# filthyrake/vlog

Hardware: AMD Instinct MI355X
Metric: audio-sec transcribed per wall-sec (RTFx), large-v3, 1/2/4/8 MI355X; WER delta (higher is better)
Workload: dtype bf16; 1 GPU; config 4: large-v3 bf16 greedy, timestamps on, 150 x 30 s windows per GPU of the seeded speech-like corpus (uniform transcript lengths), window-sharded; model=large-v3, windows_per_gpu=150, decoder_steps=113, decode=all-rows batch, decoder_row_steps=16950, corpus=uniform, parallelism=window-shard x1

## Files before the change

### vlog_amd/csrc/attn_enc.hip

```cpp
#include "common.h"
#include <cstdlib>
#include <stdexcept>
#include <string>
#include <type_traits>

#define HD 64
#define KT 64
#define VT_LD 68

__device__ __forceinline__ int kswz(int row, int ch) { return row * HD + ((ch ^ ((row >> 1) & 7)) << 3); }

__global__ __launch_bounds__(256) void attn_enc_kernel(const bf16* __restrict__ qkv, bf16* __restrict__ out, int T,
                                                       int d, float scale_log2) {
  __shared__ __attribute__((aligned(16))) bf16 sK[KT * HD];
  __shared__ __attribute__((aligned(16))) bf16 sVt[HD * VT_LD];
  const int tid = threadIdx.x, lane = tid & 63, wv = tid >> 6;
  const int g = lane >> 4, ql = lane & 15;
  const int h = blockIdx.y, b = blockIdx.z;
  const long long ld = 3LL * d;
  const bf16* base = qkv + (long long)b * T * ld;
  const int q0 = blockIdx.x * 64 + wv * 16;

  bf16x8 qf[2];
  {
    const int q = q0 + ql;
#pragma unroll
    for (int kk = 0; kk < 2; ++kk) {
      if (q < T) qf[kk] = *(const bf16x8*)(base + (long long)q * ld + h * HD + kk * 32 + 8 * g);
      else qf[kk] = bf16x8{};
    }
  }

  f32x4 o[4];
#pragma unroll
  for (int i = 0; i < 4; ++i) o[i] = f32x4{0.f, 0.f, 0.f, 0.f};
  float m_run = -INFINITY, l_run = 0.f;

  i32x4 rk[2], rv[2];
  const int nt = (T + KT - 1) / KT;
#define LOAD_TILE(t_)                                                                       \
  {                                                                                         \
    _Pragma("unroll") for (int i = 0; i < 2; ++i) {                                         \
      const int c = tid + i * 256, key = (t_) * KT + (c >> 3), ch = c & 7;                  \
      if (key < T) {                                                                        \
        const bf16* p = base + (long long)key * ld + h * HD + ch * 8;                        \
        rk[i] = *(const i32x4*)(p + d);                                                     \
        rv[i] = *(const i32x4*)(p + 2 * d);                                                 \
      } else {                                                                              \
        rk[i] = i32x4{0, 0, 0, 0};                                                          \
        rv[i] = i32x4{0, 0, 0, 0};                                                          \
      }                                                                                     \
    }                                                                                       \
  }
  LOAD_TILE(0);
  for (int t = 0; t < nt; ++t) {
    __syncthreads();
#pragma unroll
    for (int i = 0; i < 2; ++i) {
      const int c = tid + i * 256, key = c >> 3, ch = c & 7;
      *(i32x4*)(&sK[kswz(key, ch)]) = rk[i];
      bf16x8 vv = __builtin_bit_cast(bf16x8, rv[i]);
#pragma unroll
      for (int e = 0; e < 8; ++e) sVt[(ch * 8 + e) * VT_LD + key] = vv[e];
    }
    __syncthreads();
    if (t + 1 < nt) LOAD_TILE(t + 1);

    f32x4 s[4];
#pragma unroll
    for (int mi = 0; mi < 4; ++mi) {
      s[mi] = f32x4{0.f, 0.f, 0.f, 0.f};
#pragma unroll
      for (int kk = 0; kk < 2; ++kk) {
        const bf16x8 ka = *(const bf16x8*)(&sK[kswz(mi * 16 + ql, kk * 4 + g)]);
        s[mi] = __builtin_amdgcn_mfma_f32_16x16x32_bf16(ka, qf[kk], s[mi], 0, 0, 0);
      }
    }
    float tmax = -INFINITY;
    const int kbase = t * KT;
#pragma unroll
    for (int mi = 0; mi < 4; ++mi)
#pragma unroll
      for (int e = 0; e < 4; ++e) {
        const int key = kbase + mi * 16 + 4 * g + e;
        float v = s[mi][e] * scale_log2;
        if (key >= T) v = -INFINITY;
        s[mi][e] = v;
        tmax = fmaxf(tmax, v);
      }
    tmax = fmaxf(tmax, __shfl_xor(tmax, 16, 64));
    tmax = fmaxf(tmax, __shfl_xor(tmax, 32, 64));
    const float m_new = fmaxf(m_run, tmax);
    const float alpha = exp2f(m_run - m_new);
    float psum = 0.f;
#pragma unroll
    for (int mi = 0; mi < 4; ++mi)
#pragma unroll
      for (int e = 0; e < 4; ++e) {
        const float p = exp2f(s[mi][e] - m_new);
        s[mi][e] = p;
        psum += p;
      }
    psum += __shfl_xor(psum, 16, 64);
    psum += __shfl_xor(psum, 32, 64);
    l_run = l_run * alpha + psum;
    m_run = m_new;
#pragma unroll
    for (int ni = 0; ni < 4; ++ni) o[ni] *= alpha;

#pragma unroll
    for (int ks = 0; ks < 2; ++ks) {
      bf16x8 pb;
#pragma unroll
      for (int e = 0; e < 4; ++e) {
        pb[e] = f2bf(s[2 * ks][e]);
        pb[4 + e] = f2bf(s[2 * ks + 1][e]);
      }
#pragma unroll
      for (int ni = 0; ni < 4; ++ni) {
        const bf16* vr = &sVt[(ni * 16 + ql) * VT_LD + ks * 32 + 4 * g];
        const bf16x4 lo = *(const bf16x4*)(vr);
        const bf16x4 hi = *(const bf16x4*)(vr + 16);
        bf16x8 va;
#pragma unroll
        for (int e = 0; e < 4; ++e) { va[e] = lo[e]; va[4 + e] = hi[e]; }
        o[ni] = __builtin_amdgcn_mfma_f32_16x16x32_bf16(va, pb, o[ni], 0, 0, 0);
      }
    }
  }
#undef LOAD_TILE

  const int q = q0 + ql;
  if (q < T) {
    const float inv = 1.0f / l_run;
    bf16* orow = out + ((long long)b * T + q) * d + h * HD;
#pragma unroll
    for (int ni = 0; ni < 4; ++ni) {
      bf16x4 w;
#pragma unroll
      for (int e = 0; e < 4; ++e) w[e] = f2bf(o[ni][e] * inv);
      *(bf16x4*)(orow + ni * 16 + 4 * g) = w;
    }
  }
}

#define A2_KT 64
#define A2_THR 8.0f
typedef __attribute__((ext_vector_type(4))) short i16x4;
typedef __attribute__((ext_vector_type(2))) int i32x2;

__device__ __forceinline__ int a2_kslot(int r, int c) { return r * 64 + ((c ^ ((r >> 1) & 7)) << 3); }
__device__ __forceinline__ int a2_vslot(int r, int c) { return r * 64 + ((c ^ (((r >> 1) & 1) << 2)) << 3); }

__global__ __launch_bounds__(256, 2) void attn_enc_v2_kernel(const bf16* __restrict__ qkv, bf16* __restrict__ out,
                                                             int T, int d, float scale_log2, int n_head) {
  __shared__ __attribute__((aligned(16))) bf16 smem[2 * 2 * A2_KT * HD];
  const int tid = threadIdx.x, lane = tid & 63, wv = tid >> 6;
  const int ql = lane & 31, hh = lane >> 5;
  const int nqt = (T + 127) / 128;
  int qt, h, b;
  {
    const int nwg = gridDim.x, bid = blockIdx.x, xcd = bid & 7, q8 = nwg >> 3, r8 = nwg & 7;
    const int wgid = (xcd < r8 ? xcd * (q8 + 1) : r8 * (q8 + 1) + (xcd - r8) * q8) + (bid >> 3);
    qt = wgid % nqt;
    const int rest = wgid / nqt;
    h = rest % n_head;
    b = rest / n_head;
  }
  const long long ld = 3LL * d;
  const bf16* base = qkv + (long long)b * T * ld + h * HD;
  const int q = qt * 128 + wv * 32 + ql;

  bf16x8 qf[4];
  {
    const int qc = min(q, T - 1);
#pragma unroll
    for (int s = 0; s < 4; ++s) {
      const bf16x8 v = *(const bf16x8*)(base + (long long)qc * ld + 16 * s + 8 * hh);
#pragma unroll
      for (int j = 0; j < 8; ++j) qf[s][j] = f2bf(bf2f(v[j]) * scale_log2);
    }
  }
  f32x16 o[2];
#pragma unroll
  for (int i = 0; i < 2; ++i)
#pragma unroll
    for (int r = 0; r < 16; ++r) o[i][r] = 0.f;
  float m_run = -INFINITY, l_run = 0.f;

  i32x4 rk[2], rv[2];
  const int nt = (T + A2_KT - 1) / A2_KT;
  auto load_tile = [&](int t) {
#pragma unroll
    for (int i = 0; i < 2; ++i) {
      const int c = tid + i * 256, key = min(t * A2_KT + (c >> 3), T - 1), ch = c & 7;
      const bf16* p = base + (long long)key * ld + ch * 8;
      rk[i] = *(const i32x4*)(p + d);
      rv[i] = *(const i32x4*)(p + 2 * d);
    }
  };
  auto store_tile = [&](int buf) {
    bf16* sK = smem + buf * (2 * A2_KT * HD);
    bf16* sV = sK + A2_KT * HD;
#pragma unroll
    for (int i = 0; i < 2; ++i) {
      const int c = tid + i * 256, r = c >> 3, ch = c & 7;
      *(i32x4*)(sK + a2_kslot(r, ch)) = rk[i];
      *(i32x4*)(sV + a2_vslot(r, ch)) = rv[i];
    }
  };
  load_tile(0);
  store_tile(0);
  __syncthreads();

  const int G = lane >> 4, gi = lane & 15, gq = gi >> 2, gp = gi & 3;
  for (int t = 0; t < nt; ++t) {
    const bf16* sK = smem + (t & 1) * (2 * A2_KT * HD);
    const bf16* sV = sK + A2_KT * HD;
    if (t + 1 < nt) load_tile(t + 1);

    f32x16 sc[2];
#pragma unroll
    for (int kb = 0; kb < 2; ++kb) {
#pragma unroll
      for (int r = 0; r < 16; ++r) sc[kb][r] = 0.f;
#pragma unroll
      for (int s = 0; s < 4; ++s) {
        const bf16x8 ka = *(const bf16x8*)(sK + a2_kslot(kb * 32 + ql, 2 * s + hh));
        sc[kb] = __builtin_amdgcn_mfma_f32_32x32x16_bf16(ka, qf[s], sc[kb], 0, 0, 0);
      }
    }
    if (t == nt - 1) {
#pragma unroll
      for (int kb = 0; kb < 2; ++kb)
#pragma unroll
        for (int r = 0; r < 16; ++r) {
          const int key = t * A2_KT + kb * 32 + 8 * (r >> 2) + 4 * hh + (r & 3);
          if (key >= T) sc[kb][r] = -INFINITY;
        }
    }
    float mx = sc[0][0];
#pragma unroll
    for (int kb = 0; kb < 2; ++kb)
#pragma unroll
      for (int r = 0; r < 16; ++r) mx = fmaxf(mx, sc[kb][r]);
    mx = fmaxf(mx, __shfl_xor(mx, 32, 64));
    if (__any(mx > m_run + A2_THR)) {
      const float mn = fmaxf(m_run, mx);
      const float alpha = __builtin_amdgcn_exp2f(m_run - mn);
      l_run *= alpha;
#pragma unroll
      for (int i = 0; i < 2; ++i)
#pragma unroll
        for (int r = 0; r < 16; ++r) o[i][r] *= alpha;
      m_run = mn;
    }
    bf16x8 pf[2][2];
#pragma unroll
    for (int kb = 0; kb < 2; ++kb)
#pragma unroll
      for (int r = 0; r < 16; ++r) {
        const float pv = __builtin_amdgcn_exp2f(sc[kb][r] - m_run);
        l_run += pv;
        pf[kb][r >> 3][r & 7] = f2bf(pv);
      }
#pragma unroll
    for (int kb = 0; kb < 2; ++kb)
#pragma unroll
      for (int s = 0; s < 2; ++s)
#pragma unroll
        for (int hb = 0; hb < 2; ++hb) {
          bf16x8 va;
#ifndef A2_SCALAR_V
          i32x2 vw[2];
#endif
#pragma unroll
          for (int jh = 0; jh < 2; ++jh) {
            const int row = kb * 32 + 16 * s + 8 * jh + 4 * (G >> 1) + gq;
            const int col = 32 * hb + 16 * (G & 1) + 4 * gp;
#ifdef A2_SCALAR_V
            const int rowb = row - gq, hdc = 32 * hb + 16 * (G & 1) + gi;
#pragma unroll
            for (int e = 0; e < 4; ++e) va[4 * jh + e] = sV[a2_vslot(rowb + e, hdc >> 3) + (hdc & 7)];
#else
            const bf16* ad = sV + a2_vslot(row, col >> 3) + (col & 7);
            vw[jh] = __builtin_bit_cast(i32x2, __builtin_amdgcn_ds_read_tr16_b64_v4i16(
                                                   (__attribute__((address_space(3))) i16x4*)(ad)));
#endif
          }
#ifndef A2_SCALAR_V
          va = __builtin_bit_cast(bf16x8, i32x4{vw[0][0], vw[0][1], vw[1][0], vw[1][1]});
#endif
          o[hb] = __builtin_amdgcn_mfma_f32_32x32x16_bf16(va, pf[kb][s], o[hb], 0, 0, 0);
        }
    if (t + 1 < nt) store_tile((t + 1) & 1);
    __syncthreads();
  }

  l_run += __shfl_xor(l_run, 32, 64);
  if (q < T) {
    const float inv = 1.0f / l_run;
    bf16* orow = out + ((long long)b * T + q) * d + h * HD;
#pragma unroll
    for (int hb = 0; hb < 2; ++hb)
#pragma unroll
      for (int g = 0; g < 4; ++g) {
        bf16x4 w;
#pragma unroll
        for (int e = 0; e < 4; ++e) w[e] = f2bf(o[hb][4 * g + e] * inv);
        *(bf16x4*)(orow + 32 * hb + 8 * g + 4 * hh) = w;
      }
  }
}

__device__ __forceinline__ void a3_scores(const bf16* sK, const bf16x8 (&qf)[4], int ql, int hh, f32x16 (&sc)[2]) {
#pragma unroll
  for (int kb = 0; kb < 2; ++kb)
#pragma unroll
    for (int r = 0; r < 16; ++r) sc[kb][r] = 0.f;
#pragma unroll
  for (int s = 0; s < 4; ++s)
#pragma unroll
    for (int kb = 0; kb < 2; ++kb) {
      const bf16x8 ka = *(const bf16x8*)(sK + a2_kslot(kb * 32 + ql, 2 * s + hh));
      sc[kb] = __builtin_amdgcn_mfma_f32_32x32x16_bf16(ka, qf[s], sc[kb], 0, 0, 0);
    }
}

__global__ __launch_bounds__(256, 2) void attn_enc_v3_kernel(const bf16* __restrict__ qkv, bf16* __restrict__ out,
                                                             int T, int d, float scale_log2, int n_head) {
  __shared__ __attribute__((aligned(16))) bf16 smem[3 * 2 * A2_KT * HD];
  const int tid = threadIdx.x, lane = tid & 63, wv = tid >> 6;
  const int ql = lane & 31, hh = lane >> 5;
  const int nqt = (T + 127) / 128;
  int qt, h, b;
  {
    const int nwg = gridDim.x, bid = blockIdx.x, xcd = bid & 7, q8 = nwg >> 3, r8 = nwg & 7;
    const int wgid = (xcd < r8 ? xcd * (q8 + 1) : r8 * (q8 + 1) + (xcd - r8) * q8) + (bid >> 3);
    qt = wgid % nqt;
    const int rest = wgid / nqt;
    h = rest % n_head;
    b = rest / n_head;
  }
  const long long ld = 3LL * d;
  const bf16* base = qkv + (long long)b * T * ld + h * HD;
  const int q = qt * 128 + wv * 32 + ql;

  bf16x8 qf[4];
  {
    const int qc = min(q, T - 1);
#pragma unroll
    for (int s = 0; s < 4; ++s) {
      const bf16x8 v = *(const bf16x8*)(base + (long long)qc * ld + 16 * s + 8 * hh);
#pragma unroll
      for (int j = 0; j < 8; ++j) qf[s][j] = f2bf(bf2f(v[j]) * scale_log2);
    }
  }
  f32x16 o[2];
#pragma unroll
  for (int i = 0; i < 2; ++i)
#pragma unroll
    for (int r = 0; r < 16; ++r) o[i][r] = 0.f;
  float m_run = -INFINITY, l_run = 0.f;

  i32x4 rk[2], rv[2];
  const int nt = (T + A2_KT - 1) / A2_KT;
  auto load_tile = [&](int t) {
#pragma unroll
    for (int i = 0; i < 2; ++i) {
      const int c = tid + i * 256, key = min(t * A2_KT + (c >> 3), T - 1), ch = c & 7;
      const bf16* p = base + (long long)key * ld + ch * 8;
      rk[i] = *(const i32x4*)(p + d);
      rv[i] = *(const i32x4*)(p + 2 * d);
    }
  };
  auto store_tile = [&](int slot) {
    bf16* sK = smem + slot * (2 * A2_KT * HD);
    bf16* sV = sK + A2_KT * HD;
#pragma unroll
    for (int i = 0; i < 2; ++i) {
      const int c = tid + i * 256, r = c >> 3, ch = c & 7;
      *(i32x4*)(sK + a2_kslot(r, ch)) = rk[i];
      *(i32x4*)(sV + a2_vslot(r, ch)) = rv[i];
    }
  };
  load_tile(0);
  store_tile(0);
  if (nt > 1) {
    load_tile(1);
    store_tile(1);
  }
  __syncthreads();

  const int G = lane >> 4, gi = lane & 15, gq = gi >> 2, gp = gi & 3;
  f32x16 sc[2];
  a3_scores(smem, qf, ql, hh, sc);

  auto tile = [&](int t, int slot, auto last_tag) {
    constexpr bool LAST = decltype(last_tag)::value;
    const bf16* sV = smem + slot * (2 * A2_KT * HD) + A2_KT * HD;
    f32x16 sn[2];
    if constexpr (!LAST) load_tile(t + 2);
    if constexpr (LAST) {
#pragma unroll
      for (int kb = 0; kb < 2; ++kb)
#pragma unroll
        for (int r = 0; r < 16; ++r) {
          const int key = t * A2_KT + kb * 32 + 8 * (r >> 2) + 4 * hh + (r & 3);
          if (key >= T) sc[kb][r] = -INFINITY;
        }
    }
    float mx = sc[0][0];
#pragma unroll
    for (int kb = 0; kb < 2; ++kb)
#pragma unroll
      for (int r = 0; r < 16; ++r) mx = fmaxf(mx, sc[kb][r]);
    mx = fmaxf(mx, __shfl_xor(mx, 32, 64));
    if (__any(mx > m_run + A2_THR)) {
      const float mn = fmaxf(m_run, mx);
      const float alpha = __builtin_amdgcn_exp2f(m_run - mn);
      l_run *= alpha;
#pragma unroll
      for (int i = 0; i < 2; ++i)
#pragma unroll
        for (int r = 0; r < 16; ++r) o[i][r] *= alpha;
      m_run = mn;
    }
    if constexpr (!LAST) a3_scores(smem + (slot == 2 ? 0 : slot + 1) * (2 * A2_KT * HD), qf, ql, hh, sn);
    bf16x8 pf[2][2];
#pragma unroll
    for (int kb = 0; kb < 2; ++kb)
#pragma unroll
      for (int r = 0; r < 16; ++r) {
        const float pv = __builtin_amdgcn_exp2f(sc[kb][r] - m_run);
        l_run += pv;
        pf[kb][r >> 3][r & 7] = f2bf(pv);
      }
#pragma unroll
    for (int kb = 0; kb < 2; ++kb)
#pragma unroll
      for (int s = 0; s < 2; ++s)
#pragma unroll
        for (int hb = 0; hb < 2; ++hb) {
          i32x2 vw[2];
#pragma unroll
          for (int jh = 0; jh < 2; ++jh) {
            const int row = kb * 32 + 16 * s + 8 * jh + 4 * (G >> 1) + gq;
            const int col = 32 * hb + 16 * (G & 1) + 4 * gp;
            const bf16* ad = sV + a2_vslot(row, col >> 3) + (col & 7);
            vw[jh] = __builtin_bit_cast(i32x2, __builtin_amdgcn_ds_read_tr16_b64_v4i16(
                                                   (__attribute__((address_space(3))) i16x4*)(ad)));
          }
          const bf16x8 va = __builtin_bit_cast(bf16x8, i32x4{vw[0][0], vw[0][1], vw[1][0], vw[1][1]});
          o[hb] = __builtin_amdgcn_mfma_f32_32x32x16_bf16(va, pf[kb][s], o[hb], 0, 0, 0);
        }
    if constexpr (!LAST) {
      store_tile(slot == 0 ? 2 : slot - 1);
      __syncthreads();
#pragma unroll
      for (int kb = 0; kb < 2; ++kb) sc[kb] = sn[kb];
    }
  };
  int slot = 0;
  for (int t = 0; t < nt - 1; ++t) {
    tile(t, slot, std::false_type{});
    slot = slot == 2 ? 0 : slot + 1;
  }
  tile(nt - 1, slot, std::true_type{});

  l_run += __shfl_xor(l_run, 32, 64);
  if (q < T) {
    const float inv = 1.0f / l_run;
    bf16* orow = out + ((long long)b * T + q) * d + h * HD;
#pragma unroll
    for (int hb = 0; hb < 2; ++hb)
#pragma unroll
      for (int g = 0; g < 4; ++g) {
        bf16x4 w;
#pragma unroll
        for (int e = 0; e < 4; ++e) w[e] = f2bf(o[hb][4 * g + e] * inv);
        *(bf16x4*)(orow + 32 * hb + 8 * g + 4 * hh) = w;
      }
  }
}

static int attn_enc_form() {
  static const int v = [] {
    const char* e1 = std::getenv("VLOG_AMD_ATTN_V1");
    if (e1 && e1[0] == '1') return 1;
    const char* e = std::getenv("VLOG_AMD_ATTN_V");
    const int f = e ? std::atoi(e) : 2;
    return (f >= 1 && f <= 3) ? f : 2;
  }();
  return v;
}

void launch_attn_enc(const bf16* qkv, bf16* out, int B, int T, int d, int n_head, hipStream_t st) {
  if (B <= 0) return;
  if (d != n_head * HD) throw std::runtime_error("attn_enc: head_dim must be 64");
  const float scale_log2 = 0.125f * 1.4426950408889634f;
  const int form = attn_enc_form();
  if (form == 1) {
    dim3 grid((T + 63) / 64, n_head, B);
    hipLaunchKernelGGL(attn_enc_kernel, grid, dim3(256), 0, st, qkv, out, T, d, scale_log2);
  } else {
    const long long nblk = (long long)((T + 127) / 128) * n_head * B;
    if (nblk > (1LL << 31) - 1) throw std::runtime_error("attn_enc: grid too large");
    if (form == 3)
      hipLaunchKernelGGL(attn_enc_v3_kernel, dim3((unsigned)nblk), dim3(256), 0, st, qkv, out, T, d, scale_log2, n_head);
    else
      hipLaunchKernelGGL(attn_enc_v2_kernel, dim3((unsigned)nblk), dim3(256), 0, st, qkv, out, T, d, scale_log2, n_head);
  }
  WM_LAUNCH_CHECK("attn_enc_kernel");
}
```

Before: 3888 audio_s/s.

## Add v4 encoder attention with buffer loads, double-buffering and tail skipping

Replaces the v1 and v3 encoder attention kernels with a new default v4 kernel. It loads K/V through buffer resource loads with scalar offsets, so clamping and bounds checks are done by the hardware. It uses a 2-slot LDS double buffer with compile-time buffer indices and drops v3's score prefetching. It also skips fully out-of-range waves and the unused half of the last key tile. Encoder time should drop through less address arithmetic and wasted tail work, but losing v3's score/PV overlap may reduce latency hiding.

```diff
diff --git a/vlog_amd/csrc/attn_enc.hip b/vlog_amd/csrc/attn_enc.hip
--- a/vlog_amd/csrc/attn_enc.hip
+++ b/vlog_amd/csrc/attn_enc.hip
@@ -5,144 +5,6 @@
 #include <type_traits>
 
 #define HD 64
-#define KT 64
-#define VT_LD 68
-
-__device__ __forceinline__ int kswz(int row, int ch) { return row * HD + ((ch ^ ((row >> 1) & 7)) << 3); }
-
-__global__ __launch_bounds__(256) void attn_enc_kernel(const bf16* __restrict__ qkv, bf16* __restrict__ out, int T,
-                                                       int d, float scale_log2) {
-  __shared__ __attribute__((aligned(16))) bf16 sK[KT * HD];
-  __shared__ __attribute__((aligned(16))) bf16 sVt[HD * VT_LD];
-  const int tid = threadIdx.x, lane = tid & 63, wv = tid >> 6;
-  const int g = lane >> 4, ql = lane & 15;
-  const int h = blockIdx.y, b = blockIdx.z;
-  const long long ld = 3LL * d;
-  const bf16* base = qkv + (long long)b * T * ld;
-  const int q0 = blockIdx.x * 64 + wv * 16;
-
-  bf16x8 qf[2];
-  {
-    const int q = q0 + ql;
-#pragma unroll
-    for (int kk = 0; kk < 2; ++kk) {
-      if (q < T) qf[kk] = *(const bf16x8*)(base + (long long)q * ld + h * HD + kk * 32 + 8 * g);
-      else qf[kk] = bf16x8{};
-    }
-  }
-
-  f32x4 o[4];
-#pragma unroll
-  for (int i = 0; i < 4; ++i) o[i] = f32x4{0.f, 0.f, 0.f, 0.f};
-  float m_run = -INFINITY, l_run = 0.f;
-
-  i32x4 rk[2], rv[2];
-  const int nt = (T + KT - 1) / KT;
-#define LOAD_TILE(t_)                                                                       \
-  {                                                                                         \
-    _Pragma("unroll") for (int i = 0; i < 2; ++i) {                                         \
-      const int c = tid + i * 256, key = (t_) * KT + (c >> 3), ch = c & 7;                  \
-      if (key < T) {                                                                        \
-        const bf16* p = base + (long long)key * ld + h * HD + ch * 8;                        \
-        rk[i] = *(const i32x4*)(p + d);                                                     \
-        rv[i] = *(const i32x4*)(p + 2 * d);                                                 \
-      } else {                                                                              \
-        rk[i] = i32x4{0, 0, 0, 0};                                                          \
-        rv[i] = i32x4{0, 0, 0, 0};                                                          \
-      }                                                                                     \
-    }                                                                                       \
-  }
-  LOAD_TILE(0);
-  for (int t = 0; t < nt; ++t) {
-    __syncthreads();
-#pragma unroll
-    for (int i = 0; i < 2; ++i) {
-      const int c = tid + i * 256, key = c >> 3, ch = c & 7;
-      *(i32x4*)(&sK[kswz(key, ch)]) = rk[i];
-      bf16x8 vv = __builtin_bit_cast(bf16x8, rv[i]);
-#pragma unroll
-      for (int e = 0; e < 8; ++e) sVt[(ch * 8 + e) * VT_LD + key] = vv[e];
-    }
-    __syncthreads();
-    if (t + 1 < nt) LOAD_TILE(t + 1);
-
-    f32x4 s[4];
-#pragma unroll
-    for (int mi = 0; mi < 4; ++mi) {
-      s[mi] = f32x4{0.f, 0.f, 0.f, 0.f};
-#pragma unroll
-      for (int kk = 0; kk < 2; ++kk) {
-        const bf16x8 ka = *(const bf16x8*)(&sK[kswz(mi * 16 + ql, kk * 4 + g)]);
-        s[mi] = __builtin_amdgcn_mfma_f32_16x16x32_bf16(ka, qf[kk], s[mi], 0, 0, 0);
-      }
-    }
-    float tmax = -INFINITY;
-    const int kbase = t * KT;
-#pragma unroll
-    for (int mi = 0; mi < 4; ++mi)
-#pragma unroll
-      for (int e = 0; e < 4; ++e) {
-        const int key = kbase + mi * 16 + 4 * g + e;
-        float v = s[mi][e] * scale_log2;
-        if (key >= T) v = -INFINITY;
-        s[mi][e] = v;
-        tmax = fmaxf(tmax, v);
-      }
-    tmax = fmaxf(tmax, __shfl_xor(tmax, 16, 64));
-    tmax = fmaxf(tmax, __shfl_xor(tmax, 32, 64));
-    const float m_new = fmaxf(m_run, tmax);
-    const float alpha = exp2f(m_run - m_new);
-    float psum = 0.f;
-#pragma unroll
-    for (int mi = 0; mi < 4; ++mi)
-#pragma unroll
-      for (int e = 0; e < 4; ++e) {
-        const float p = exp2f(s[mi][e] - m_new);
-        s[mi][e] = p;
-        psum += p;
-      }
-    psum += __shfl_xor(psum, 16, 64);
-    psum += __shfl_xor(psum, 32, 64);
-    l_run = l_run * alpha + psum;
-    m_run = m_new;
-#pragma unroll
-    for (int ni = 0; ni < 4; ++ni) o[ni] *= alpha;
-
-#pragma unroll
-    for (int ks = 0; ks < 2; ++ks) {
-      bf16x8 pb;
-#pragma unroll
-      for (int e = 0; e < 4; ++e) {
-        pb[e] = f2bf(s[2 * ks][e]);
-        pb[4 + e] = f2bf(s[2 * ks + 1][e]);
-      }
-#pragma unroll
-      for (int ni = 0; ni < 4; ++ni) {
-        const bf16* vr = &sVt[(ni * 16 + ql) * VT_LD + ks * 32 + 4 * g];
-        const bf16x4 lo = *(const bf16x4*)(vr);
-        const bf16x4 hi = *(const bf16x4*)(vr + 16);
-        bf16x8 va;
-#pragma unroll
-        for (int e = 0; e < 4; ++e) { va[e] = lo[e]; va[4 + e] = hi[e]; }
-        o[ni] = __builtin_amdgcn_mfma_f32_16x16x32_bf16(va, pb, o[ni], 0, 0, 0);
-      }
-    }
-  }
-#undef LOAD_TILE
-
-  const int q = q0 + ql;
-  if (q < T) {
-    const float inv = 1.0f / l_run;
-    bf16* orow = out + ((long long)b * T + q) * d + h * HD;
-#pragma unroll
-    for (int ni = 0; ni < 4; ++ni) {
-      bf16x4 w;
-#pragma unroll
-      for (int e = 0; e < 4; ++e) w[e] = f2bf(o[ni][e] * inv);
-      *(bf16x4*)(orow + ni * 16 + 4 * g) = w;
-    }
-  }
-}
 
 #define A2_KT 64
 #define A2_THR 8.0f
@@ -313,24 +175,19 @@
   }
 }
 
-__device__ __forceinline__ void a3_scores(const bf16* sK, const bf16x8 (&qf)[4], int ql, int hh, f32x16 (&sc)[2]) {
-#pragma unroll
-  for (int kb = 0; kb < 2; ++kb)
-#pragma unroll
-    for (int r = 0; r < 16; ++r) sc[kb][r] = 0.f;
-#pragma unroll
-  for (int s = 0; s < 4; ++s)
-#pragma unroll
-    for (int kb = 0; kb < 2; ++kb) {
-      const bf16x8 ka = *(const bf16x8*)(sK + a2_kslot(kb * 32 + ql, 2 * s + hh));
-      sc[kb] = __builtin_amdgcn_mfma_f32_32x32x16_bf16(ka, qf[s], sc[kb], 0, 0, 0);
-    }
-}
-
-__global__ __launch_bounds__(256, 2) void attn_enc_v3_kernel(const bf16* __restrict__ qkv, bf16* __restrict__ out,
+
+__device__ __forceinline__ __amdgpu_buffer_rsrc_t a4_rsrc(const bf16* base, int T, int d) {
+  return __builtin_amdgcn_make_buffer_rsrc((void*)base, 0, (((T - 1) * 3 + 2) * d + HD) * 2, 0x00020000);
+}
+__device__ __forceinline__ i32x4 a4_load(__amdgpu_buffer_rsrc_t rsrc, int voff, int soff) {
+  return __builtin_bit_cast(i32x4, __builtin_amdgcn_raw_buffer_load_b128(rsrc, voff, soff, 0));
+}
+
+__global__ __launch_bounds__(256, 2) void attn_enc_v4_kernel(const bf16* __restrict__ qkv, bf16* __restrict__ out,
                                                              int T, int d, float scale_log2, int n_head) {
-  __shared__ __attribute__((aligned(16))) bf16 smem[3 * 2 * A2_KT * HD];
-  const int tid = threadIdx.x, lane = tid & 63, wv = tid >> 6;
+  __shared__ __attribute__((aligned(16))) bf16 smem[2 * 2 * A2_KT * HD];
+  const int tid = threadIdx.x, lane = tid & 63;
+  const int wv = __builtin_amdgcn_readfirstlane(tid >> 6);
   const int ql = lane & 31, hh = lane >> 5;
   const int nqt = (T + 127) / 128;
   int qt, h, b;
@@ -345,6 +202,9 @@
   const long long ld = 3LL * d;
   const bf16* base = qkv + (long long)b * T * ld + h * HD;
   const int q = qt * 128 + wv * 32 + ql;
+  const bool active = qt * 128 + wv * 32 < T;
+  const int nt = (T + A2_KT - 1) / A2_KT;
+  const bool skip1 = (nt - 1) * A2_KT + 32 >= T;
 
   bf16x8 qf[4];
   {
@@ -364,112 +224,135 @@
   float m_run = -INFINITY, l_run = 0.f;
 
   i32x4 rk[2], rv[2];
-  const int nt = (T + A2_KT - 1) / A2_KT;
+  const __amdgpu_buffer_rsrc_t rsrc = a4_rsrc(base, T, d);
+  const int sr = tid >> 3, sch = tid & 7;
+  const int voff = (sr * 3 * d + sch * 8) * 2;
   auto load_tile = [&](int t) {
 #pragma unroll
     for (int i = 0; i < 2; ++i) {
-      const int c = tid + i * 256, key = min(t * A2_KT + (c >> 3), T - 1), ch = c & 7;
-      const bf16* p = base + (long long)key * ld + ch * 8;
-      rk[i] = *(const i32x4*)(p + d);
-      rv[i] = *(const i32x4*)(p + 2 * d);
-    }
-  };
-  auto store_tile = [&](int slot) {
-    bf16* sK = smem + slot * (2 * A2_KT * HD);
+      const int so = (t * A2_KT + 32 * i) * 3 * d * 2;
+      rk[i] = a4_load(rsrc, voff, so + d * 2);
+      rv[i] = a4_load(rsrc, voff, so + 2 * d * 2);
+    }
+  };
+  auto store_tile = [&](int buf) {
+    bf16* sK = smem + buf * (2 * A2_KT * HD);
     bf16* sV = sK + A2_KT * HD;
 #pragma unroll
     for (int i = 0; i < 2; ++i) {
-      const int c = tid + i * 256, r = c >> 3, ch = c & 7;
-      *(i32x4*)(sK + a2_kslot(r, ch)) = rk[i];
-      *(i32x4*)(sV + a2_vslot(r, ch)) = rv[i];
+      *(i32x4*)(sK + a2_kslot(sr + 32 * i, sch)) = rk[i];
+      *(i32x4*)(sV + a2_vslot(sr + 32 * i, sch)) = rv[i];
     }
   };
   load_tile(0);
   store_tile(0);
-  if (nt > 1) {
-    load_tile(1);
-    store_tile(1);
-  }
   __syncthreads();
 
   const int G = lane >> 4, gi = lane & 15, gq = gi >> 2, gp = gi & 3;
-  f32x16 sc[2];
-  a3_scores(smem, qf, ql, hh, sc);
-
-  auto tile = [&](int t, int slot, auto last_tag) {
+  auto tile = [&](int t, auto buf_tag, auto last_tag) {
+    constexpr int BUF = decltype(buf_tag)::value;
     constexpr bool LAST = decltype(last_tag)::value;
-    const bf16* sV = smem + slot * (2 * A2_KT * HD) + A2_KT * HD;
-    f32x16 sn[2];
-    if constexpr (!LAST) load_tile(t + 2);
-    if constexpr (LAST) {
-#pragma unroll
-      for (int kb = 0; kb < 2; ++kb)
+    const bf16* sK = smem + BUF * (2 * A2_KT * HD);
+    const bf16* sV = sK + A2_KT * HD;
+    const int nkb = LAST && skip1 ? 1 : 2;
+    if constexpr (!LAST) load_tile(t + 1);
+    if (active) {
+      f32x16 sc[2];
+#pragma unroll
+      for (int kb = 0; kb < 2; ++kb) {
+        if (kb >= nkb) break;
+#pragma unroll
+        for (int r = 0; r < 16; ++r) sc[kb][r] = 0.f;
+#pragma unroll
+        for (int s = 0; s < 4; ++s) {
+          const bf16x8 ka = *(const bf16x8*)(sK + a2_kslot(kb * 32 + ql, 2 * s + hh));
+          sc[kb] = __builtin_amdgcn_mfma_f32_32x32x16_bf16(ka, qf[s], sc[kb], 0, 0, 0);
+        }
+      }
+      if constexpr (LAST) {
+#pragma unroll
+        for (int kb = 0; kb < 2; ++kb) {
+          if (kb >= nkb) break;
+#pragma unroll
+          for (int r = 0; r < 16; ++r) {
+            const int key = t * A2_KT + kb * 32 + 8 * (r >> 2) + 4 * hh + (r & 3);
+            if (key >= T) sc[kb][r] = -INFINITY;
+          }
+        }
+      }
+      float mx = sc[0][0];
+#pragma unroll
+      for (int kb = 0; kb < 2; ++kb) {
+        if (kb >= nkb) break;
+#pragma unroll
+        for (int r = 0; r < 16; ++r) mx = fmaxf(mx, sc[kb][r]);
+      }
+      mx = fmaxf(mx, __shfl_xor(mx, 32, 64));
+      if (__any(mx > m_run + A2_THR)) {
+        const float mn = fmaxf(m_run, mx);
+        const float alpha = __builtin_amdgcn_exp2f(m_run - mn);
+        l_run *= alpha;
+#pragma unroll
+        for (int i = 0; i < 2; ++i)
+#pragma unroll
+          for (int r = 0; r < 16; ++r) o[i][r] *= alpha;
+        m_run = mn;
+      }
+      bf16x8 pf[2][2];
+#pragma unroll
+      for (int kb = 0; kb < 2; ++kb) {
+        if (kb >= nkb) break;
 #pragma unroll
         for (int r = 0; r < 16; ++r) {
-          const int key = t * A2_KT + kb * 32 + 8 * (r >> 2) + 4 * hh + (r & 3);
-          if (key >= T) sc[kb][r] = -INFINITY;
-        }
-    }
-    float mx = sc[0][0];
-#pragma unroll
-    for (int kb = 0; kb < 2; ++kb)
-#pragma unroll
-      for (int r = 0; r < 16; ++r) mx = fmaxf(mx, sc[kb][r]);
-    mx = fmaxf(mx, __shfl_xor(mx, 32, 64));
-    if (__any(mx > m_run + A2_THR)) {
-      const float mn = fmaxf(m_run, mx);
-      const float alpha = __builtin_amdgcn_exp2f(m_run - mn);
-      l_run *= alpha;
-#pragma unroll
-      for (int i = 0; i < 2; ++i)
-#pragma unroll
-        for (int r = 0; r < 16; ++r) o[i][r] *= alpha;
-      m_run = mn;
-    }
-    if constexpr (!LAST) a3_scores(smem + (slot == 2 ? 0 : slot + 1) * (2 * A2_KT * HD), qf, ql, hh, sn);
-    bf16x8 pf[2][2];
-#pragma unroll
-    for (int kb = 0; kb < 2; ++kb)
-#pragma unroll
-      for (int r = 0; r < 16; ++r) {
-        const float pv = __builtin_amdgcn_exp2f(sc[kb][r] - m_run);
-        l_run += pv;
-        pf[kb][r >> 3][r & 7] = f2bf(pv);
-      }
-#pragma unroll
-    for (int kb = 0; kb < 2; ++kb)
-#pragma unroll
-      for (int s = 0; s < 2; ++s)
-#pragma unroll
-        for (int hb = 0; hb < 2; ++hb) {
-          i32x2 vw[2];
-#pragma unroll
-          for (int jh = 0; jh < 2; ++jh) {
-            const int row = kb * 32 + 16 * s + 8 * jh + 4 * (G >> 1) + gq;
-            const int col = 32 * hb + 16 * (G & 1) + 4 * gp;
-            const bf16* ad = sV + a2_vslot(row, col >> 3) + (col & 7);
-            vw[jh] = __builtin_bit_cast(i32x2, __builtin_amdgcn_ds_read_tr16_b64_v4i16(
-                                                   (__attribute__((address_space(3))) i16x4*)(ad)));
+          const float pv = __builtin_amdgcn_exp2f(sc[kb][r] - m_run);
+          l_run += pv;
+          pf[kb][r >> 3][r & 7] = f2bf(pv);
+        }
+      }
+#pragma unroll
+      for (int kb = 0; kb < 2; ++kb) {
+        if (kb >= nkb) break;
+#pragma unroll
+        for (int s = 0; s < 2; ++s)
+#pragma unroll
+          for (int hb = 0; hb < 2; ++hb) {
+            i32x2 vw[2];
+#pragma unroll
+            for (int jh = 0; jh < 2; ++jh) {
+              const int row = kb * 32 + 16 * s + 8 * jh + 4 * (G >> 1) + gq;
+              const int col = 32 * hb + 16 * (G & 1) + 4 * gp;
+              const bf16* ad = sV + a2_vslot(row, col >> 3) + (col & 7);
+              vw[jh] = __builtin_bit_cast(i32x2, __builtin_amdgcn_ds_read_tr16_b64_v4i16(
+                                                     (__attribute__((address_space(3))) i16x4*)(ad)));
+            }
+            const bf16x8 va = __builtin_bit_cast(bf16x8, i32x4{vw[0][0], vw[0][1], vw[1][0], vw[1][1]});
+            o[hb] = __builtin_amdgcn_mfma_f32_32x32x16_bf16(va, pf[kb][s], o[hb], 0, 0, 0);
           }
-          const bf16x8 va = __builtin_bit_cast(bf16x8, i32x4{vw[0][0], vw[0][1], vw[1][0], vw[1][1]});
-          o[hb] = __builtin_amdgcn_mfma_f32_32x32x16_bf16(va, pf[kb][s], o[hb], 0, 0, 0);
-        }
+      }
+    }
     if constexpr (!LAST) {
-      store_tile(slot == 0 ? 2 : slot - 1);
+      store_tile(BUF ^ 1);
       __syncthreads();
-#pragma unroll
-      for (int kb = 0; kb < 2; ++kb) sc[kb] = sn[kb];
-    }
-  };
-  int slot = 0;
-  for (int t = 0; t < nt - 1; ++t) {
-    tile(t, slot, std::false_type{});
-    slot = slot == 2 ? 0 : slot + 1;
-  }
-  tile(nt - 1, slot, std::true_type{});
+    }
+  };
+  {
+    using B0 = std::integral_constant<int, 0>;
+    using B1 = std::integral_constant<int, 1>;
+    int t = 0;
+    for (; t + 2 < nt; t += 2) {
+      tile(t, B0{}, std::false_type{});
+      tile(t + 1, B1{}, std::false_type{});
+    }
+    if (t + 1 < nt) {
+      tile(t, B0{}, std::false_type{});
+      tile(t + 1, B1{}, std::true_type{});
+    } else {
+      tile(t, B0{}, std::true_type{});
+    }
+  }
 
   l_run += __shfl_xor(l_run, 32, 64);
-  if (q < T) {
+  if (active && q < T) {
     const float inv = 1.0f / l_run;
     bf16* orow = out + ((long long)b * T + q) * d + h * HD;
 #pragma unroll
@@ -486,11 +369,8 @@
 
 static int attn_enc_form() {
   static const int v = [] {
-    const char* e1 = std::getenv("VLOG_AMD_ATTN_V1");
-    if (e1 && e1[0] == '1') return 1;
     const char* e = std::getenv("VLOG_AMD_ATTN_V");
-    const int f = e ? std::atoi(e) : 2;
-    return (f >= 1 && f <= 3) ? f : 2;
+    return e && std::atoi(e) == 2 ? 2 : 4;
   }();
   return v;
 }
@@ -499,17 +379,12 @@
   if (B <= 0) return;
   if (d != n_head * HD) throw std::runtime_error("attn_enc: head_dim must be 64");
   const float scale_log2 = 0.125f * 1.4426950408889634f;
-  const int form = attn_enc_form();
-  if (form == 1) {
-    dim3 grid((T + 63) / 64, n_head, B);
-    hipLaunchKernelGGL(attn_enc_kernel, grid, dim3(256), 0, st, qkv, out, T, d, scale_log2);
-  } else {
-    const long long nblk = (long long)((T + 127) / 128) * n_head * B;
-    if (nblk > (1LL << 31) - 1) throw std::runtime_error("attn_enc: grid too large");
-    if (form == 3)
-      hipLaunchKernelGGL(attn_enc_v3_kernel, dim3((unsigned)nblk), dim3(256), 0, st, qkv, out, T, d, scale_log2, n_head);
-    else
-      hipLaunchKernelGGL(attn_enc_v2_kernel, dim3((unsigned)nblk), dim3(256), 0, st, qkv, out, T, d, scale_log2, n_head);
-  }
+  const long long nblk = (long long)((T + 127) / 128) * n_head * B;
+  if (nblk > (1LL << 31) - 1) throw std::runtime_error("attn_enc: grid too large");
+  const bool fits32 = (long long)(T + A2_KT) * 3 * d * 2 < (1LL << 31);
+  if (attn_enc_form() == 2 || !fits32)
+    hipLaunchKernelGGL(attn_enc_v2_kernel, dim3((unsigned)nblk), dim3(256), 0, st, qkv, out, T, d, scale_log2, n_head);
+  else
+    hipLaunchKernelGGL(attn_enc_v4_kernel, dim3((unsigned)nblk), dim3(256), 0, st, qkv, out, T, d, scale_log2, n_head);
   WM_LAUNCH_CHECK("attn_enc_kernel");
 }
```

After: 3904 audio_s/s (median of 6 runs). No clear change (+0.4%).
